# denix56/SI-Mamba

Hardware: AMD Instinct MI355X
Metric: point-clouds/sec (fwd+bwd) (higher is better)
Workload: dtype f32; 1 GPU; PointMamba classifier train step (FPS+kNN grouping, encoder, spectral SAST ordering, 12 Mamba blocks d=384 at L=1024, head, AdamW), 1024 pts -> 128 patches; global_batch=64, per_gpu_batch=64, npoints=1024, patches=128, mamba_seq_len=1024, parallelism=dp1, communicator_ranks=1, library_gemm=tuned solution table (si_mamba_amd/tuned/gemm_gfx950.csv)

## Files before the change

### include/simamba.h

```cpp
#ifndef SIMAMBA_H_
#define SIMAMBA_H_

#include <stddef.h>

#ifdef __cplusplus
extern "C" {
#endif

#define SIMAMBA_ABI_VERSION 9

#define SIMAMBA_F32  0
#define SIMAMBA_BF16 1

#define SIMAMBA_OK            0
#define SIMAMBA_E_NULLPTR    -1
#define SIMAMBA_E_SHAPE      -2
#define SIMAMBA_E_DTYPE      -3
#define SIMAMBA_E_DSTATE     -4
#define SIMAMBA_E_WIDTH      -5
#define SIMAMBA_E_WORKSPACE  -6
#define SIMAMBA_E_GROUPS     -7
#define SIMAMBA_E_ALIGN      -8
#define SIMAMBA_E_VARIANT    -9
#define SIMAMBA_E_BIAS       -10
// ... 44 lines not shown
                                  const float* delta_bias, const void* dout, const float* x_ckpt,
                                  void* du, void* ddelta, float* dA, float* dB, float* dC,
                                  float* dD, void* dz, float* ddelta_bias,
                                  int batch, int dim, int seqlen, int dstate,
                                  int io_dtype, int delta_softplus, long long z_bstride,
                                  long long dz_bstride, long long bc_bstride, long long bc_nstride,
                                  long long bc_tstride, int ckpt_step, int flags, float* workspace,
                                  long long workspace_floats, void* stream);

int simamba_selective_scan_dt_fwd(const void* u, const void* xdbl, const void* wdt, const float* A, const float* D,
                                  const void* z, const float* delta_bias, void* out, float* x_ckpt, float* last_state,
                                  int batch, int dim, int seqlen, int dstate, int dt_rank, int io_dtype,
                                  long long z_bstride, long long xdbl_bstride, long long xdbl_tstride, int ckpt_step,
                                  int variant, void* stream);
int simamba_selective_scan_dt_bwd(const void* u, const void* xdbl, const void* wdt, const float* A, const float* D,
                                  const void* z, const float* delta_bias, const void* dout, const float* x_ckpt,
                                  void* du, void* ddelta, float* dA, float* dB, float* dC, float* dD, void* dz,
                                  float* ddelta_bias, int batch, int dim, int seqlen, int dstate, int dt_rank,
                                  int io_dtype, long long z_bstride, long long dz_bstride, long long xdbl_bstride,
                                  long long xdbl_tstride, void* stream);
int simamba_selective_scan_dt_bwd_ex(const void* u, const void* xdbl, const void* wdt, const float* A, const float* D,
                                     const void* z, const float* delta_bias, const void* dout, const float* x_ckpt,
                                     void* du, void* ddelta, float* dA, float* dB, float* dC, float* dD, void* dz,
                                     float* ddelta_bias, int batch, int dim, int seqlen, int dstate, int dt_rank,
                                     int io_dtype, long long z_bstride, long long dz_bstride, long long xdbl_bstride,
                                     long long xdbl_tstride, int flags, float* workspace, long long workspace_floats,
                                     void* stream);

int simamba_xdt_proj_fwd(const void* x, const void* wx, const void* wdt, void* xdbl, void* delta,
                         int batch, int D, int seqlen, int S, int R, int io_dtype, long long x_bstride,
                         void* stream);
int simamba_conv_xdt_proj_fwd(const void* x, const float* cw, const float* cb, const void* wx, const void* wdt,
                              void* xconv, void* xdbl, void* delta, int batch, int D, int seqlen, int S, int R,
                              int io_dtype, long long x_bstride, void* stream);

int simamba_seq_gather_fwd(const void* in, const int* idx, void* out, int batch, int channels, int G, int L,
                           long long out_bstride, int io_dtype, void* stream);
int simamba_seq_gather_bwd(const void* dout, const int* inv, void* din, int batch, int channels, int G, int L,
                           int R, long long dout_bstride, int io_dtype, void* stream);

int simamba_causal_conv1d_fwd(const void* x, const float* w, const float* bias, void* out,
                              int batch, int dim, int seqlen, int width, int silu,
                              int io_dtype, long long x_bstride, void* stream);
int simamba_causal_conv1d_bwd(const void* x, const float* w, const float* bias,
                              const void* dout, void* dx, float* dw, float* dbias,
                              int batch, int dim, int seqlen, int width, int silu,
                              int io_dtype, long long x_bstride, long long dx_bstride, void* stream);
long long simamba_causal_conv1d_bwd_workspace_floats(int batch, int dim, int seqlen, int width, int flags);
int simamba_causal_conv1d_bwd_ex(const void* x, const float* w, const float* bias,
                                 const void* dout, void* dx, float* dw, float* dbias,
                                 int batch, int dim, int seqlen, int width, int silu,
                                 int io_dtype, long long x_bstride, long long dx_bstride, int flags,
                                 float* workspace, long long workspace_floats, void* stream);

int simamba_add_layer_norm_grid(int batch, int rows_per_batch);
int simamba_add_layer_norm_fwd(const void* hidden, const float* residual, const float* rowscale,
                               const float* weight, const float* bias, float* residual_out,
                               void* normed, float* mean, float* rstd, int batch, int rows_per_batch,
                               int dim, float eps, int hidden_dtype, int out_dtype, void* stream);
int simamba_add_layer_norm_bwd(const void* dnormed, const float* dresidual_out,
                               const float* residual_out, const float* mean, const float* rstd,
                               const float* weight, const float* rowscale, float* dresidual,
                               void* dhidden, float* dwb_partial, int batch, int rows_per_batch,
                               int dim, int hidden_dtype, int out_dtype, void* stream);

#define SIMAMBA_NORM_RMS 1
int simamba_add_layer_norm_fwd_ex(const void* hidden, const float* residual, const float* rowscale,
                                  const float* weight, const float* bias, float* residual_out,
                                  void* normed, float* mean, float* rstd, int batch, int rows_per_batch,
                                  int dim, float eps, int hidden_dtype, int out_dtype, int flags, void* stream);
int simamba_add_layer_norm_bwd_ex(const void* dnormed, const float* dresidual_out,
                                  const float* residual_out, const float* mean, const float* rstd,
                                  const float* weight, const float* rowscale, float* dresidual,
                                  void* dhidden, float* dwb_partial, int batch, int rows_per_batch,
                                  int dim, int hidden_dtype, int out_dtype, int flags, void* stream);

int simamba_add_layer_norm_check_slots(const int* slots_host, int batch, int compact_batch);
int simamba_add_layer_norm_fwd_slots(const void* hidden, const float* residual, const float* rowscale,
                                     const float* weight, const float* bias, float* residual_out,
                                     void* normed, float* mean, float* rstd, const int* hidden_slot,
                                     int hidden_batch, const int* normed_slot, int normed_batch, int batch,
                                     int rows_per_batch, int dim, float eps, int hidden_dtype, int out_dtype,
                                     int flags, void* stream);
int simamba_add_layer_norm_bwd_slots(const void* dnormed, const float* dresidual_out,
                                     const float* residual_out, const float* mean, const float* rstd,
                                     const float* weight, const float* rowscale, float* dresidual,
                                     void* dhidden, float* dwb_partial, const int* hidden_slot,
                                     int hidden_batch, const int* normed_slot, int normed_batch, int batch,
                                     int rows_per_batch, int dim, int hidden_dtype, int out_dtype, int flags,
                                     void* stream);

int simamba_out_proj_add_ln_fwd(const void* y, const void* w, const float* residual, const float* rowscale,
                                const float* gamma, const float* beta, float* residual_out, void* normed, float* mean,
                                float* rstd, int batch, int K, int L, int C, float eps, int out_dtype, void* stream);
int simamba_out_proj_add_ln_fwd_ex(const void* y, const void* w, const float* residual, const float* rowscale,
                                   const float* gamma, const float* beta, float* residual_out, void* normed,
                                   float* mean, float* rstd, int batch, int K, int L, int C, float eps, int out_dtype,
                                   int flags, void* stream);

int simamba_in_proj_fwd(const void* x, const void* w, void* xz, int batch, int L, int C, int M, int io_dtype,
                        void* stream);

int simamba_bn_relu_grid(long long rows);
int simamba_bn_relu_fwd(const void* x, const float* gterm, int group, const float* weight, const float* bias,
                        float* running_mean, float* running_var, float momentum, float eps, int training,
                        void* y, float* mean, float* invstd, float* partial, long long rows, int C,
// ... 212 lines not shown
```

### si_mamba_amd/_lib.py

```python
from __future__ import annotations

import ctypes
import os
from ctypes import c_char_p, c_float, c_int, c_longlong, c_size_t, c_uint, c_void_p

_HERE = os.path.dirname(os.path.abspath(__file__))
LIB_PATH = os.path.join(_HERE, "libsimamba_hip.so")

F32, BF16 = 0, 1

SPEC_SYMMETRIC = 0x01
SPEC_SELF_LOOP = 0x02
SPEC_BINARY = 0x04
SPEC_MATRIX_SYM = 0x08
SPEC_SMALLEST = 0x10
SPEC_SIGMA_MEAN = 0x20
SPEC_LARGE_G = 0x40
SPEC_MAX_G = 128
SPEC_MAX_G_LARGE = 512
CURVE_Z, CURVE_HILBERT, CURVE_TRANS, CURVE_Z_TRANS, CURVE_HILBERT_TRANS = 0, 1, 2, 2, 3
CURVE_BOX_CLOUD, CURVE_BOX_FIXED = 0, 1
CURVE_MAX_G, CURVE_MAX_K, CURVE_MAX_BITS = 8192, 8, 16

SCAN_AUTO, SCAN_ROWSCAN, SCAN_LPC2, SCAN_LPC4, SCAN_MIX = 0, 1, 2, 4, 6
# ... 10 lines not shown
DS_NONE, DS_UNIT_SPHERE = 0, 1
DS_STREAM_SHUFFLE, DS_STREAM_ROWS, DS_STREAM_CHOICE = 1, 2, 3
DS_MAX_POINTS = 8192
OPTIM_CHUNK = 4096
OPTIM_MAX_SEGMENTS, OPTIM_MAX_CHUNKS, OPTIM_MAX_GROUPS = 65536, 1 << 20, 256
OPTIM_ZERO_GRADS = 1

_P = c_void_p
_LL = c_longlong
ABI_VERSION = 9
SIGNATURES = {
    "simamba_abi_version": (c_int, []),
    "simamba_strerror": (c_char_p, [c_int]),
    "simamba_scan_num_chunks": (c_int, [c_int]),
    "simamba_scan_fwd_auto_variant": (c_int, [c_int, c_int]),
    "simamba_scan_ckpt_step": (c_int, [c_int, c_int, c_int, c_int, c_int]),
    "simamba_scan_ckpt_floats": (_LL, [c_int, c_int, c_int, c_int, c_int]),
    "simamba_scan_seq_applicable": (c_int, [c_int, c_int, c_int, c_int, c_int, c_int, c_int,
                                            c_size_t, c_size_t, c_size_t, c_size_t, _LL, _LL, _LL, _LL, _LL]),
    "simamba_selective_scan_fwd": (c_int, [_P, _P, _P, _P, _P, _P, _P, _P, _P, _P, _P,
                                           c_int, c_int, c_int, c_int, c_int, c_int,
                                           _LL, _LL, _LL, _LL, c_int, c_int, _P]),
    "simamba_selective_scan_bwd": (c_int, [_P, _P, _P, _P, _P, _P, _P, _P, _P, _P,
                                           _P, _P, _P, _P, _P, _P, _P, _P,
                                           c_int, c_int, c_int, c_int, c_int, c_int,
                                           _LL, _LL, _LL, _LL, _LL, c_int, _P]),
    "simamba_scan_bwd_workspace_floats": (_LL, [c_int, c_int, c_int, c_int, c_int, c_int]),
    "simamba_selective_scan_bwd_ex": (c_int, [_P, _P, _P, _P, _P, _P, _P, _P, _P, _P,
                                              _P, _P, _P, _P, _P, _P, _P, _P,
                                              c_int, c_int, c_int, c_int, c_int, c_int,
                                              _LL, _LL, _LL, _LL, _LL, c_int, c_int, _P, _LL, _P]),
    "simamba_selective_scan_dt_fwd": (c_int, [_P, _P, _P, _P, _P, _P, _P, _P, _P, _P,
                                              c_int, c_int, c_int, c_int, c_int, c_int,
                                              _LL, _LL, _LL, c_int, c_int, _P]),
    "simamba_selective_scan_dt_bwd": (c_int, [_P, _P, _P, _P, _P, _P, _P, _P, _P,
                                              _P, _P, _P, _P, _P, _P, _P, _P,
                                              c_int, c_int, c_int, c_int, c_int, c_int,
                                              _LL, _LL, _LL, _LL, _P]),
    "simamba_selective_scan_dt_bwd_ex": (c_int, [_P, _P, _P, _P, _P, _P, _P, _P, _P,
                                                 _P, _P, _P, _P, _P, _P, _P, _P,
                                                 c_int, c_int, c_int, c_int, c_int, c_int,
                                                 _LL, _LL, _LL, _LL, c_int, _P, _LL, _P]),
    "simamba_xdt_proj_fwd": (c_int, [_P, _P, _P, _P, _P, c_int, c_int, c_int, c_int, c_int, c_int, _LL, _P]),
    "simamba_conv_xdt_proj_fwd": (c_int, [_P, _P, _P, _P, _P, _P, _P, _P, c_int, c_int, c_int, c_int, c_int, c_int, _LL,
                                          _P]),
    "simamba_seq_gather_fwd": (c_int, [_P, _P, _P, c_int, c_int, c_int, c_int, _LL, c_int, _P]),
    "simamba_seq_gather_bwd": (c_int, [_P, _P, _P, c_int, c_int, c_int, c_int, c_int, _LL, c_int, _P]),
    "simamba_causal_conv1d_fwd": (c_int, [_P, _P, _P, _P, c_int, c_int, c_int, c_int, c_int, c_int, _LL, _P]),
    "simamba_causal_conv1d_bwd": (c_int, [_P, _P, _P, _P, _P, _P, _P,
                                          c_int, c_int, c_int, c_int, c_int, c_int, _LL, _LL, _P]),
    "simamba_causal_conv1d_bwd_workspace_floats": (_LL, [c_int, c_int, c_int, c_int, c_int]),
    "simamba_causal_conv1d_bwd_ex": (c_int, [_P, _P, _P, _P, _P, _P, _P,
                                             c_int, c_int, c_int, c_int, c_int, c_int, _LL, _LL, c_int, _P, _LL, _P]),
    "simamba_add_layer_norm_grid": (c_int, [c_int, c_int]),
    "simamba_add_layer_norm_fwd": (c_int, [_P, _P, _P, _P, _P, _P, _P, _P, _P, c_int, c_int, c_int, c_float,
                                           c_int, c_int, _P]),
    "simamba_add_layer_norm_bwd": (c_int, [_P, _P, _P, _P, _P, _P, _P, _P, _P, _P, c_int, c_int, c_int,
                                           c_int, c_int, _P]),
    "simamba_add_layer_norm_fwd_ex": (c_int, [_P, _P, _P, _P, _P, _P, _P, _P, _P, c_int, c_int, c_int, c_float,
                                              c_int, c_int, c_int, _P]),
    "simamba_add_layer_norm_bwd_ex": (c_int, [_P, _P, _P, _P, _P, _P, _P, _P, _P, _P, c_int, c_int, c_int,
                                              c_int, c_int, c_int, _P]),
    "simamba_add_layer_norm_check_slots": (c_int, [_P, c_int, c_int]),
    "simamba_add_layer_norm_fwd_slots": (c_int, [_P, _P, _P, _P, _P, _P, _P, _P, _P, _P, c_int, _P, c_int, c_int, c_int,
                                                 c_int, c_float, c_int, c_int, c_int, _P]),
    "simamba_add_layer_norm_bwd_slots": (c_int, [_P, _P, _P, _P, _P, _P, _P, _P, _P, _P, _P, c_int, _P, c_int, c_int,
                                                 c_int, c_int, c_int, c_int, c_int, _P]),
    "simamba_out_proj_add_ln_fwd": (c_int, [_P, _P, _P, _P, _P, _P, _P, _P, _P, _P, c_int, c_int, c_int, c_int, c_float,
                                            c_int, _P]),
    "simamba_out_proj_add_ln_fwd_ex": (c_int, [_P, _P, _P, _P, _P, _P, _P, _P, _P, _P, c_int, c_int, c_int, c_int,
                                               c_float, c_int, c_int, _P]),
    "simamba_in_proj_fwd": (c_int, [_P, _P, _P, c_int, c_int, c_int, c_int, c_int, _P]),
    "simamba_bn_relu_grid": (c_int, [_LL]),
    "simamba_bn_relu_fwd": (c_int, [_P, _P, c_int, _P, _P, _P, _P, c_float, c_float, c_int, _P, _P, _P, _P, _LL, c_int,
                                    _LL, c_int, _P]),
    "simamba_bn_relu_bwd": (c_int, [_P, _P, _P, c_int, _P, _P, _P, _P, _P, _P, c_int, _P, _P, _P, _LL, c_int, _LL,
                                    c_int, c_int, _P]),
    "simamba_bn_stats_local": (c_int, [_P, _P, c_int, _P, _LL, _P, _LL, c_int, _LL, c_int, _P]),
    "simamba_bn_stats_merge": (c_int, [_P, c_int, _P, _P, c_float, c_float, _P, _P, _P, c_int, _P]),
    "simamba_bn_relu_apply": (c_int, [_P, _P, c_int, _P, _P, _P, _P, _P, _LL, c_int, _LL, c_int, _P]),
    "simamba_bn_relu_bwd_sums": (c_int, [_P, _P, _P, c_int, _P, _P, _P, _P, _P, _P, _P, _LL, c_int, _LL, c_int, _P]),
    "simamba_bn_relu_bwd_dx": (c_int, [_P, _P, _P, c_int, _P, _P, _P, _P, _P, _P, _P, _P, _P, c_int, _LL, c_int, _LL,
                                       c_int, _P]),
    "simamba_group_max_fwd": (c_int, [_P, _P, _P, _LL, c_int, c_int, c_int, _P]),
    "simamba_group_max_bwd": (c_int, [_P, _P, _P, _LL, c_int, c_int, c_int, _P]),
    "simamba_max_linear_bwd_slabs": (c_int, [_LL, c_int]),
    "simamba_max_linear_bwd_dx": (c_int, [_P, _P, _P, _P, _LL, c_int, c_int, c_int, c_int, _P]),
    "simamba_max_linear_bwd_dw": (c_int, [_P, _P, _P, _P, _P, _LL, c_int, c_int, c_int, c_int, _P]),
    "simamba_three_nn": (c_int, [_P, _P, _P, _P, c_int, c_int, c_int, _P]),
    "simamba_three_interpolate_fwd": (c_int, [_P, _P, _P, _P, c_int, c_int, c_int, c_int, c_int, _P]),
    "simamba_three_interpolate_bwd": (c_int, [_P, _P, _P, _P, c_int, c_int, c_int, c_int, c_int, _P]),
    "simamba_gather_sum_scatter": (c_int, [_P, _P, _P, _P, c_int, c_int, c_int, c_int, c_int, c_int, _P]),
    "simamba_chamfer_fwd": (c_int, [_P, _P, _P, _P, _P, _LL, c_int, c_int, _P]),
    "simamba_chamfer_bwd": (c_int, [_P, _P, _P, _P, _P, _P, _LL, c_int, c_int, _P]),
    "simamba_chamfer_large_fwd": (c_int, [_P, _P, _P, _P, _P, _P, _P, _LL, c_int, c_int, _P]),
    "simamba_chamfer_large_bwd": (c_int, [_P, _P, _P, _P, _P, _P, _P, _LL, c_int, c_int, _P]),
    "simamba_chamfer_large_fwd_ex": (c_int, [_P, _P, _P, _P, _P, _P, _P, _LL, c_int, c_int, c_int, _P]),
    "simamba_chamfer_large_bwd_ex": (c_int, [_P, _P, _P, _P, _P, _P, _P, _LL, c_int, c_int, c_int, _P]),
    "simamba_chamfer_ragged_fwd": (c_int, [_P] * 9 + [_LL] + [c_int] * 6 + [_P]),
    "simamba_chamfer_ragged_bwd": (c_int, [_P] * 11 + [_LL] + [c_int] * 6 + [_P]),
    "simamba_emd_fwd": (c_int, [_P, _P, _P, _P, _P, _P, _LL, c_int, c_float, c_int, _P]),
    "simamba_sinkhorn_workspace_bytes": (c_size_t, [_LL, c_int, c_int, c_int]),
    "simamba_sinkhorn_fwd": (c_int, [_P] * 12 + [_LL, c_int, c_int, c_float, c_int, c_int, _P, c_size_t, _P]),
    "simamba_sinkhorn_bwd": (c_int, [_P] * 11 + [_LL, c_int, c_int, c_float, c_int, _P, c_size_t, _P]),
    "simamba_part_seg_eval": (c_int, [_P] * 12 + [_LL, c_int, c_int, c_int, _P]),
    "simamba_svm_ovo_fit": (c_int, [_P] * 10 + [c_int, c_int, c_int, c_int, c_int, _P]),
# ... 172 lines not shown
_scan_ckpt = [0]


class scan_ckpt(_Override):
    cell, coerce = _scan_ckpt, int

    def __init__(self, step):
        super().__init__(step)


_spectral_large_g = [False]


class spectral_large_g(_Override):
    cell = _spectral_large_g

    def __init__(self, on=True):
        super().__init__(on)


def spectral_large_g_forced():
    return _spectral_large_g[0]


_fuse_dt = [None]
counters = {}


def count(name):
    counters[name] = counters.get(name, 0) + 1


class scan_fuse_dt(_Override):
    cell, coerce = _fuse_dt, staticmethod(_tristate)


def fuse_dt_enabled(dtype):
    import torch
    return (dtype == torch.bfloat16) if _fuse_dt[0] is None else _fuse_dt[0]


_fuse_out_norm = [True]
_hand_in_proj = [None]


class fuse_out_norm(_Override):
    cell = _fuse_out_norm


def fuse_out_norm_enabled():
    return _fuse_out_norm[0]


_drop_path_compact = [os.environ.get("SIMAMBA_DROP_PATH_COMPACT", "1").strip().lower() not in ("0", "false", "off")]
DROP_PATH_BUCKET = 4
compact_sizes = {}


class drop_path_compact(_Override):
    cell = _drop_path_compact


def drop_path_compact_enabled():
    return _drop_path_compact[0]


_sparse_max_linear = [None]


class sparse_max_linear(_Override):
    cell, coerce = _sparse_max_linear, staticmethod(_tristate)


def sparse_max_linear_enabled(dtype):
    import torch
    return (dtype == torch.float32) if _sparse_max_linear[0] is None else _sparse_max_linear[0]


class hand_in_proj(_Override):
    cell, coerce = _hand_in_proj, staticmethod(_tristate)


def in_proj_hand_enabled(workgroups, dtype=None):
    import torch
    if _hand_in_proj[0] is not None:
        return _hand_in_proj[0]
    return dtype != torch.float32 and workgroups >= IN_PROJ_MIN_WORKGROUPS


IN_PROJ_MIN_WORKGROUPS = 192


def scan_plan_step(batch, dim, seqlen, dstate, dtype, *, softplus=True, has_z=True, act_addr_or=0, a_addr=0,
                   b_addr=0, c_addr=0, z_bs=0, dz_bs=0, bc_strides=(0, 0, 0)):
    lib = load()
    code = dtype_code(dtype)
    step = _scan_ckpt[0] or lib.simamba_scan_ckpt_step(batch, dim, seqlen, dstate, code)
    if step == CKPT_SEQ and not lib.simamba_scan_seq_applicable(
            batch, dim, seqlen, dstate, code, int(bool(softplus)), int(bool(has_z)), act_addr_or, a_addr, b_addr,
            c_addr, z_bs, dz_bs, *bc_strides):
        step = CKPT_ROW
    if _scan_variant[0] == SCAN_ROWSCAN:
        step = CKPT_ROW
    return step


# ... 59 lines not shown
```

### si_mamba_amd/add_norm.py

```python
from __future__ import annotations

import torch

from . import _lib


def add_norm_bwd(dn, dro, res_out, mean, rstd, w, rs, dres, dhid, Bsz, rows, dim, hcode, ocode, flags,
                 hidden_slot=None, hidden_batch=None, normed_slot=None, normed_batch=None):
    dev = res_out.device
    grid = _lib.load().simamba_add_layer_norm_grid(Bsz, rows)
    part = torch.empty(grid, 2, dim, device=dev, dtype=torch.float32)
    hb = Bsz if hidden_slot is None else hidden_batch
    nb = Bsz if normed_slot is None else normed_batch
    _lib.call("simamba_add_layer_norm_bwd_slots", dn, dro, res_out, mean, rstd, w, rs, dres, dhid, part, hidden_slot, hb,
              normed_slot, nb, Bsz, rows, dim, hcode, ocode, flags, device=dev,
              time_as="add_rms_bwd" if flags else "add_ln_bwd")
    return part[:, :1].sum(0) if flags else part.sum(0)


class AddLayerNormFn(torch.autograd.Function):
    @staticmethod
    def forward(ctx, hidden, residual, weight, bias, eps, rowscale, out_dtype, rms=False, hidden_slot=None,
                hidden_dtype=None, normed_slot=None, normed_batch=None):
        full = hidden if hidden_slot is None else residual
        if full is None:
            raise ValueError("add_layer_norm_fn: a compact hidden (hidden_slot) goes with a residual")
        _lib.require_gpu(full, "add_layer_norm_fn")
        h = None if hidden is None else hidden.contiguous()
        Bsz, rows, dim = full.shape[0], full[0].numel() // full.shape[-1], full.shape[-1]
        shape = tuple(full.shape)
        dev = full.device
        hdtype = h.dtype if h is not None else (hidden_dtype or torch.float32)
        hb = Bsz if hidden_slot is None else (0 if h is None else h.shape[0])
        nb = Bsz if normed_slot is None else int(normed_batch)
        if h is not None and tuple(h.shape[1:]) != shape[1:]:
            raise ValueError(f"add_layer_norm_fn: hidden {tuple(h.shape)} against residual {shape}")
        hcode = _lib.dtype_code(hdtype)
        ocode = _lib.dtype_code(out_dtype)
        flags = _lib.NORM_RMS if rms else 0
        res = None if residual is None else residual.float().contiguous()
        w = weight.float().contiguous()
        b = None if bias is None else bias.float().contiguous()
        rs = None if (rowscale is None or res is None) else rowscale.float().contiguous()
        alias = res is None and hdtype == torch.float32
        res_out = h if alias else torch.empty(shape, device=dev, dtype=torch.float32)
        normed = torch.empty((nb,) + shape[1:], device=dev, dtype=out_dtype)
        mean = None if rms else torch.empty(Bsz * rows, device=dev, dtype=torch.float32)
        rstd = torch.empty(Bsz * rows, device=dev, dtype=torch.float32)
        _lib.call("simamba_add_layer_norm_fwd_slots", h, res, rs, w, b, None if alias else res_out, normed, mean, rstd,
                  hidden_slot, hb, normed_slot, nb, Bsz, rows, dim, float(eps), hcode, ocode, flags, device=dev,
                  time_as="add_rms_fwd" if rms else "add_ln_fwd")
        ctx.save_for_backward(res_out, mean, rstd, w, rs, hidden_slot, normed_slot)
        ctx.meta = (Bsz, rows, dim, hcode, ocode, hdtype, residual is not None,
                    None if residual is None else residual.dtype, weight.dtype, bias is not None, flags, hb, nb)
        return normed, res_out

    @staticmethod
    def backward(ctx, dnormed, dres_out):
        res_out, mean, rstd, w, rs, hidden_slot, normed_slot = ctx.saved_tensors
        Bsz, rows, dim, hcode, ocode, hdtype, has_res, res_dtype, wdtype, has_bias, flags, hb, nb = ctx.meta
        dev = res_out.device
        dn = dnormed.contiguous()
        dro = None if dres_out is None else dres_out.float().contiguous()
        need_split = (rs is not None) or (hdtype != torch.float32) or not has_res or hidden_slot is not None
        dres = torch.empty(res_out.shape, device=dev, dtype=torch.float32) if has_res else None
        dhid = torch.empty((hb,) + tuple(res_out.shape[1:]), device=dev, dtype=hdtype) if need_split and hb else None
        dwb = add_norm_bwd(dn, dro, res_out, mean, rstd, w, rs, dres, dhid, Bsz, rows, dim, hcode, ocode, flags,
                           hidden_slot, hb, normed_slot, nb)
        if dhid is None and hidden_slot is None:
            dhid = dres
# ... 19 lines not shown
```

### si_mamba_amd/csrc/api.hip

```cpp
#include <hip/hip_runtime.h>

#include "../../include/simamba.h"

extern "C" int simamba_abi_version(void) { return SIMAMBA_ABI_VERSION; }

extern "C" const char* simamba_strerror(int rc) {
  switch (rc) {
    case SIMAMBA_OK: return "ok";
    case SIMAMBA_E_NULLPTR: return "simamba: required pointer is NULL";
    case SIMAMBA_E_SHAPE: return "simamba: bad shape (negative size, dim <= 0 or batch > 65535)";
    case SIMAMBA_E_DTYPE: return "simamba: io_dtype must be SIMAMBA_F32 or SIMAMBA_BF16";
    case SIMAMBA_E_DSTATE: return "simamba: dstate must be in [1,16]";
    case SIMAMBA_E_WIDTH: return "simamba: conv width must be in [2,4]";
    case SIMAMBA_E_WORKSPACE: return "simamba: workspace missing or too small";
    case SIMAMBA_E_GROUPS: return "simamba: need 2 <= G <= 128 (512 for the graph, _ex and fused calls), knn + 1 <= min(G, 32), k (+1) <= G (<= 8 above 128), 1 <= F <= 64";
    case SIMAMBA_E_ALIGN: return "simamba: pointer not aligned";
    case SIMAMBA_E_VARIANT: return "simamba: scan variant unknown or not applicable to this shape, unknown flag bits, or an augmentation chain / buffer overlap the call cannot take";
    case SIMAMBA_E_BIAS: return "simamba: SIMAMBA_NORM_RMS takes no bias / beta (pass NULL)";
    default: break;
  }
  if (rc > 0) return hipGetErrorString(static_cast<hipError_t>(rc));
  return "simamba: unknown error code";
}
```

### si_mamba_amd/csrc/det_reduce.h

```cpp
#pragma once
#include <hip/hip_runtime.h>

namespace simamba {

struct DetSumJob {
  const float* part;
  float* out;
  long long kstride;
  long long n;
  int K;
};

constexpr int kDetSumMaxJobs = 5;

int det_sum_launch(const DetSumJob* jobs, int njobs, hipStream_t s);

}
```

### si_mamba_amd/csrc/det_reduce.hip

```cpp
#include "det_reduce.h"

namespace simamba {

constexpr int kDetSumThreads = 256;
constexpr int kDetSumPerBlock = 4 * kDetSumThreads;

struct DetSumArgs {
  DetSumJob job[kDetSumMaxJobs];
  int vec[kDetSumMaxJobs];
  int blk0[kDetSumMaxJobs + 1];
  int njobs;
};

__global__ __launch_bounds__(kDetSumThreads) void det_sum_kernel(DetSumArgs a) {
  const int blk = blockIdx.x;
  int j = 0;
#pragma unroll
  for (int q = 1; q < kDetSumMaxJobs; ++q) j = (q < a.njobs && blk >= a.blk0[q]) ? q : j;
  const float* __restrict__ part = a.job[j].part;
  float* __restrict__ out = a.job[j].out;
  const long long ks = a.job[j].kstride, n = a.job[j].n;
  const int K = a.job[j].K;
  const long long i0 = (static_cast<long long>(blk - a.blk0[j]) * kDetSumThreads + threadIdx.x) * 4;
  if (i0 >= n) return;
  if (a.vec[j] && i0 + 4 <= n) {
    const float* p = part + i0;
    float4 acc = make_float4(0.f, 0.f, 0.f, 0.f);
    int k = 0;
    for (; k + 4 <= K; k += 4) {
      float4 v[4];
#pragma unroll
      for (int m = 0; m < 4; ++m) v[m] = *reinterpret_cast<const float4*>(p + (k + m) * ks);
#pragma unroll
      for (int m = 0; m < 4; ++m) {
        acc.x += v[m].x; acc.y += v[m].y; acc.z += v[m].z; acc.w += v[m].w;
      }
    }
    for (; k < K; ++k) {
      const float4 v = *reinterpret_cast<const float4*>(p + k * ks);
      acc.x += v.x; acc.y += v.y; acc.z += v.z; acc.w += v.w;
    }
    *reinterpret_cast<float4*>(out + i0) = acc;
    return;
  }
  for (long long i = i0; i < n && i < i0 + 4; ++i) {
    float acc = 0.f;
    for (int k = 0; k < K; ++k) acc += part[k * ks + i];
    out[i] = acc;
  }
}

int det_sum_launch(const DetSumJob* jobs, int njobs, hipStream_t s) {
  DetSumArgs a{};
  int blocks = 0, m = 0;
  for (int i = 0; i < njobs && m < kDetSumMaxJobs; ++i) {
    if (jobs[i].n <= 0) continue;
    a.job[m] = jobs[i];
    a.vec[m] = (reinterpret_cast<uintptr_t>(jobs[i].part) & 15u) == 0 && (reinterpret_cast<uintptr_t>(jobs[i].out) & 15u) == 0 &&
               jobs[i].kstride % 4 == 0;
    a.blk0[m] = blocks;
    blocks += static_cast<int>((jobs[i].n + kDetSumPerBlock - 1) / kDetSumPerBlock);
    ++m;
  }
  if (!m) return static_cast<int>(hipSuccess);
  a.njobs = m;
  for (int q = m; q <= kDetSumMaxJobs; ++q) a.blk0[q] = blocks;
  hipLaunchKernelGGL(det_sum_kernel, dim3(blocks), dim3(kDetSumThreads), 0, s, a);
  return static_cast<int>(hipGetLastError());
}

}
```

### si_mamba_amd/encoder_ops.py

```python
from __future__ import annotations

import torch
import torch.distributed as dist

from . import _lib


_BN_MAX_C = 1024
_BN_CHUNK = 256


_SPLITK = 64
_SPLITK_MIN_ROWS = 512


class TokenLinearFn(torch.autograd.Function):

    @staticmethod
    def forward(ctx, x, weight, bias):
        y = torch.nn.functional.linear(x, weight, bias)
        ctx.save_for_backward(x, weight)
        ctx.has_bias = bias is not None
        return y

    @staticmethod
    def backward(ctx, dy):
        x, weight = ctx.saved_tensors
        dy = dy.contiguous()
        io = dy.dtype
        rows, n_out = dy.shape
        dx = dw = db = None
        if ctx.needs_input_grad[0]:
            dx = (dy @ weight.to(io)).to(x.dtype)
        if ctx.needs_input_grad[1]:
            xc = x.to(io).contiguous()
            if rows % _SPLITK == 0 and rows // _SPLITK >= _SPLITK_MIN_ROWS:
                m = rows // _SPLITK
                a = dy.view(_SPLITK, m, n_out).transpose(1, 2)
                b = xc.view(_SPLITK, m, xc.shape[1])
                part = torch.bmm(a, b) if io == torch.float32 else torch.bmm(a, b, out_dtype=torch.float32)
                dw = part.sum(0).to(weight.dtype)
            else:
                dw = (dy.t() @ xc).to(weight.dtype)
        if ctx.has_bias and ctx.needs_input_grad[2]:
            db = dy.sum(0, dtype=torch.float32).to(weight.dtype)
        return dx, dw, db


def token_linear(x, weight, bias=None):
    if x.is_cuda and x.dim() == 2 and torch.is_grad_enabled() and (weight.requires_grad or x.requires_grad):
        return TokenLinearFn.apply(x, weight, bias)
    return torch.nn.functional.linear(x, weight, bias)


def _slices(C):
    return [(c0, min(c0 + _BN_MAX_C, C)) for c0 in range(0, C, _BN_MAX_C)]


def _off(t, elems):
    return None if t is None else t.data_ptr() + elems * t.element_size()


def _slice_of(g, c0, c1, C):
    return None if g is None else (g if (c0 == 0 and c1 == C) else g[:, c0:c1].contiguous())


def _bn_partial(lib, rows, C, dev):
    return torch.empty(lib.simamba_bn_relu_grid(rows), 2, min(C, _BN_MAX_C), device=dev, dtype=torch.float32)


def _bn_operands(x, gterm, weight, bias):
    xc = x.contiguous()
    g, w, b = (None if t is None else t.float().contiguous() for t in (gterm, weight, bias))
    mean = torch.empty(xc.shape[1], device=xc.device, dtype=torch.float32)
    return xc, g, w, b, torch.empty_like(xc), mean, torch.empty_like(mean)


def _dtypes(*tensors):
    return tuple(None if t is None else t.dtype for t in tensors)


def _bn_grads(dtypes, dx, dgt, dw, db):
    xdtype, gdtype, wdtype, bdtype = dtypes
    return (dx.to(xdtype), None if dgt is None else dgt.to(gdtype), None,
            None if wdtype is None else dw.to(wdtype), None if bdtype is None else db.to(bdtype),
            None, None, None, None, None)


def _bn_dgroup(g, group):
    dgroup = 0 if g is None else (group if _BN_CHUNK % group == 0 else _BN_CHUNK)
    if g is not None and dgroup == _BN_CHUNK and group % _BN_CHUNK != 0:
        raise ValueError("bn_relu_fn: group must divide 256 or be a multiple of it")
    return dgroup

# ... 298 lines not shown
```

### si_mamba_amd/mamba_inner.py

```python
from __future__ import annotations

import torch

from . import _lib


def _w(t, dtype):
    return t if t.dtype == dtype else t.to(dtype)


def _wx(W, X):
    return torch.bmm(W.unsqueeze(0).expand(X.shape[0], -1, -1), X)


def _xw(X, W):
    return torch.bmm(X, W.unsqueeze(0).expand(X.shape[0], -1, -1))


def _sum_bmm(X, Y):
    return torch.bmm(X, Y).sum(0, dtype=torch.float32)


class InProjFn(torch.autograd.Function):

    @staticmethod
    def forward(ctx, hidden, weight, bias):
        io = hidden.dtype
        if torch.is_autocast_enabled("cuda"):
            io = torch.get_autocast_dtype("cuda")
            hidden = hidden.to(io)
        wc = _w(weight, io)
        xz = tokens_times_weight(hidden, wc) if bias is None else _wx(wc, hidden.transpose(1, 2))
        if bias is not None:
            xz = xz + _w(bias, io)[None, :, None]
        ctx.save_for_backward(hidden, weight)
        ctx.wc = wc
        ctx.has_bias = bias is not None
        return xz

    @staticmethod
    def backward(ctx, dxz):
        hidden, weight = ctx.saved_tensors
        io = hidden.dtype
        dxz = dxz.to(io)
        dh = _xw(dxz.transpose(1, 2), ctx.wc) if ctx.needs_input_grad[0] else None
        dw = _sum_bmm(dxz, hidden).to(weight.dtype) if ctx.needs_input_grad[1] else None
        db = dxz.sum((0, 2)).to(weight.dtype) if ctx.has_bias else None
        return dh, dw, db


def tokens_times_weight(x, w):
    if (x.dtype in (torch.bfloat16, torch.float32) and w.dtype == x.dtype and x.is_cuda and x.dim() == 3
            and x.is_contiguous() and in_proj_hand_ok(x, w)):
        Bsz, L, C = x.shape
        wcc = w.contiguous()
        out = torch.empty(Bsz, w.shape[0], L, device=x.device, dtype=x.dtype)
        _lib.call("simamba_in_proj_fwd", x, wcc, out, Bsz, L, C, w.shape[0], _lib.dtype_code(x.dtype),
                  device=x.device, time_as="in_proj_fwd")
        _lib.count("in_proj_hand")
        return out
    return _wx(w, x.transpose(1, 2))


def in_proj_hand_ok(hidden, wc):
    Bsz, L, C = hidden.shape
    tile = 128 if hidden.dtype == torch.float32 else 256
    return (C % 64 == 0 and C <= 384 and wc.shape[0] % 32 == 0 and L % 8 == 0 and hidden.data_ptr() % 16 == 0
            and _lib.in_proj_hand_enabled(Bsz * ((L + tile - 1) // tile), hidden.dtype))


def in_proj_fn(hidden, weight, bias=None):
    return InProjFn.apply(hidden, weight, bias)

# ... 75 lines not shown
                x_dbl = _xw(x_conv.transpose(1, 2), xw_c.t())
                delta = _wx(dtw_c, x_dbl[:, :, :R].transpose(1, 2))
        Bv, Cv = x_dbl[:, :, R:R + N], x_dbl[:, :, R + N:]
        if x_dbl.data_ptr() % 16 or not x_dbl.is_contiguous():
            raise RuntimeError("mamba_inner_fn: x_proj output not as planned")

        y = torch.empty(Bsz, Dm, L, device=dev, dtype=io)
        dtw_k = dtw_c.contiguous() if fuse_dt else None
        if fuse_dt:
            _lib.count("scan_dt_fwd")
            _lib.call("simamba_selective_scan_dt_fwd", x_conv, x_dbl, dtw_k, Af, Df, z, bf, y, x_ckpt, None,
                      Bsz, Dm, L, N, R, code, xbs, x_dbl.stride(0), x_dbl.stride(1),
                      ckpt_step, _lib.current_scan_variant(), device=dev, time_as="scan_fwd")
        else:
            _lib.call("simamba_selective_scan_fwd", x_conv, delta, Af, Bv, Cv, Df, z, bf, y, x_ckpt, None,
                      Bsz, Dm, L, N, code, 1, xbs, x_dbl.stride(0), 1, x_dbl.stride(1),
                      ckpt_step, _lib.current_scan_variant(), device=dev, time_as="scan_fwd")

        if no_out:
            out = y
        else:
            out = _xw(y.transpose(1, 2), ow_c.t())
            if out_proj_b is not None:
                out = out + _w(out_proj_b, io)
        ctx.no_out = no_out
        ctx.dims = (R, N, W)
        ctx.ckpt_step = ckpt_step
        ctx.dtw_k = dtw_k
        ctx.has_out_bias = out_proj_b is not None and not no_out
        ctx.param_dtypes = (conv_w.dtype, None if conv_b is None else conv_b.dtype, x_proj_w.dtype,
                            dt_proj_w.dtype, None if no_out else out_proj_w.dtype, A.dtype,
                            None if D is None else D.dtype, None if delta_bias is None else delta_bias.dtype)
        ctx.save_for_backward(xz, x_conv, x_dbl, delta, None if no_out else y, cw, cb, x_proj_w, dt_proj_w, out_proj_w,
                              Af, Df, bf, x_ckpt)
        return out

    @staticmethod
    def backward(ctx, dout):
        (xz, x_conv, x_dbl, delta, y, cw, cb, x_proj_w, dt_proj_w, out_proj_w, Af, Df, bf, x_ckpt) = ctx.saved_tensors
        lib = _lib.load()
        R, N, W = ctx.dims
        io = xz.dtype
        code = _lib.dtype_code(io)
        Bsz, twoD, L = xz.shape
        Dm = twoD // 2
        S = R + 2 * N
        dev = xz.device
        xbs = xz.stride(0)
        dout = dout.to(io)
        f32 = dict(device=dev, dtype=torch.float32)
        xw_c, dtw_c, ow_c = ctx.wcast
        if ctx.no_out:
            dy = dout.contiguous()
            d_out_w = d_out_b = None
        else:
            if dout.stride(2) != 1:
                dout = dout.contiguous()
            d_out_w = _sum_bmm(dout.transpose(1, 2), y.transpose(1, 2))
            d_out_b = dout.sum((0, 1)) if ctx.has_out_bias else None
            dy = tokens_times_weight(dout, ow_c.t())

        dxz = torch.empty_like(xz)
        du = torch.empty(Bsz, Dm, L, device=dev, dtype=io)
        ddelta = torch.empty(Bsz, Dm, L, device=dev, dtype=io)
        dA, dB, dC, dD, dbias = _lib.scan_bwd_accumulators(Bsz, Dm, L, N, Df is not None, bf is not None, dev)
        Bv, Cv = x_dbl[:, :, R:R + N], x_dbl[:, :, R + N:]
        z, dz = xz[:, Dm:], dxz[:, Dm:]
        flags, ws, nws = _lib.det_args(lib.simamba_scan_bwd_workspace_floats, Bsz, Dm, L, N,
                                       _lib.CKPT_SEQ if ctx.dtw_k is not None else ctx.ckpt_step, device=dev)
        _lib.count("scan_bwd_det" if flags else "scan_bwd_atomic")
        if ctx.dtw_k is not None:
            _lib.call("simamba_selective_scan_dt_bwd_ex", x_conv, x_dbl, ctx.dtw_k, Af, Df, z, bf, dy, x_ckpt,
                      du, ddelta, dA, dB, dC, dD, dz, dbias, Bsz, Dm, L, N, R, code,
                      xbs, dxz.stride(0), x_dbl.stride(0), x_dbl.stride(1), flags, ws, nws,
                      device=dev, time_as="scan_bwd")
        else:
            _lib.call("simamba_selective_scan_bwd_ex", x_conv, delta, Af, Bv, Cv, Df, z, bf, dy, x_ckpt,
                      du, ddelta, dA, dB, dC, dD, dz, dbias, Bsz, Dm, L, N, code, 1,
                      xbs, dxz.stride(0), x_dbl.stride(0), 1, x_dbl.stride(1), ctx.ckpt_step, flags, ws, nws,
                      device=dev, time_as="scan_bwd")

        dx_dbl = torch.empty(Bsz, L, S, device=dev, dtype=io)
        dx_dbl[:, :, :R].copy_(_xw(ddelta.transpose(1, 2), dtw_c))
        dBC = torch.as_strided(dB, (2, Bsz, N, L), (Bsz * N * L, N * L, L, 1))
        dx_dbl[:, :, R:].view(Bsz, L, 2, N).copy_(dBC.permute(1, 3, 0, 2))
        d_dt_w = _sum_bmm(ddelta, x_dbl[:, :, :R])
        d_x_w = _sum_bmm(dx_dbl.transpose(1, 2), x_conv.transpose(1, 2))
        wxT = xw_c.t().unsqueeze(0).expand(Bsz, -1, -1)
        torch.baddbmm(du, wxT, dx_dbl.transpose(1, 2), out=du)

        dconv = torch.empty(Dm * W + (Dm if cb is not None else 0), **f32)
        dcw = dconv[:Dm * W].view(Dm, W)
        dcb = dconv[Dm * W:] if cb is not None else None
        flags, ws, nws = _lib.det_args(lib.simamba_causal_conv1d_bwd_workspace_floats, Bsz, Dm, L, W, device=dev)
        _lib.count("conv1d_bwd_det" if flags else "conv1d_bwd_atomic")
        _lib.call("simamba_causal_conv1d_bwd_ex", xz, cw, cb, du, dxz, dcw, dcb, Bsz, Dm, L, W, 1, code,
                  xbs, dxz.stride(0), flags, ws, nws, device=dev, time_as="conv1d_bwd")

        t_cw, t_cb, t_xw, t_dtw, t_ow, t_A, t_D, t_b = ctx.param_dtypes
        return (dxz, dcw.to(t_cw), None if dcb is None else dcb.to(t_cb), d_x_w.to(t_xw), d_dt_w.to(t_dtw),
                None if d_out_w is None else d_out_w.to(t_ow),
                None if d_out_b is None else d_out_b.to(out_proj_w.dtype), dA.to(t_A),
                None if dD is None else dD.to(t_D), None if dbias is None else dbias.to(t_b), None, None, None)


def mamba_inner_fn(xz, conv1d_weight, conv1d_bias, x_proj_weight, delta_proj_weight, out_proj_weight,
                   out_proj_bias, A, D=None, delta_bias=None, dt_rank=None, d_state=None):
    if conv1d_weight.dim() == 3:
        conv1d_weight = conv1d_weight.squeeze(1)
    if dt_rank is None:
        dt_rank = delta_proj_weight.shape[1]
    if d_state is None:
        d_state = (x_proj_weight.shape[0] - dt_rank) // 2
    return MambaInnerFn.apply(xz, conv1d_weight, conv1d_bias, x_proj_weight, delta_proj_weight, out_proj_weight,
                              out_proj_bias, A, D, delta_bias, dt_rank, d_state, torch.is_grad_enabled())
```

Measured before the change: 1177 point-clouds/s.

## Replace per-batch bmm partial sums with a fused multi-job deterministic batch_sum kernel

Adds a simamba_batch_sum entry point that reduces up to five per-batch partial tensors over the leading dimension in one launch, with f32/bf16 inputs and a split-K scheme that spreads each reduction across several threads followed by an LDS combine. The weight-gradient reductions in the mamba backward (out_proj, x_proj, dt_proj), the encoder split-K dw and the add-norm partials now call this kernel instead of separate torch sum calls. The aim is to cut launch count and use more of the GPU on these small reductions. It adds ctypes marshaling overhead on each call, and keeping p_out_w alive longer raises peak memory slightly.

```diff
diff --git a/include/simamba.h b/include/simamba.h
--- a/include/simamba.h
+++ b/include/simamba.h
@@ -120,6 +120,10 @@
                                  int batch, int dim, int seqlen, int width, int silu,
                                  int io_dtype, long long x_bstride, long long dx_bstride, int flags,
                                  float* workspace, long long workspace_floats, void* stream);
+
+#define SIMAMBA_BATCH_SUM_MAX_JOBS 5
+int simamba_batch_sum(const void* const* parts, float* const* outs, const long long* kstrides, const long long* ns,
+                      const int* Ks, const int* part_dtypes, int njobs, void* stream);
 
 int simamba_add_layer_norm_grid(int batch, int rows_per_batch);
 int simamba_add_layer_norm_fwd(const void* hidden, const float* residual, const float* rowscale,
diff --git a/si_mamba_amd/_lib.py b/si_mamba_amd/_lib.py
--- a/si_mamba_amd/_lib.py
+++ b/si_mamba_amd/_lib.py
@@ -86,6 +86,7 @@
     "simamba_causal_conv1d_bwd_workspace_floats": (_LL, [c_int, c_int, c_int, c_int, c_int]),
     "simamba_causal_conv1d_bwd_ex": (c_int, [_P, _P, _P, _P, _P, _P, _P,
                                              c_int, c_int, c_int, c_int, c_int, c_int, _LL, _LL, c_int, _P, _LL, _P]),
+    "simamba_batch_sum": (c_int, [_P, _P, _P, _P, _P, _P, c_int, _P]),
     "simamba_add_layer_norm_grid": (c_int, [c_int, c_int]),
     "simamba_add_layer_norm_fwd": (c_int, [_P, _P, _P, _P, _P, _P, _P, _P, _P, c_int, c_int, c_int, c_float,
                                            c_int, c_int, _P]),
@@ -364,6 +365,21 @@
     return _fuse_out_norm[0]
 
 
+_aten_batch_sum = [False]
+BATCH_SUM_MAX_JOBS = 5
+
+
+class aten_batch_sum(_Override):
+    cell = _aten_batch_sum
+
+    def __init__(self, on=True):
+        super().__init__(on)
+
+
+def aten_batch_sum_forced():
+    return _aten_batch_sum[0]
+
+
 _drop_path_compact = [os.environ.get("SIMAMBA_DROP_PATH_COMPACT", "1").strip().lower() not in ("0", "false", "off")]
 DROP_PATH_BUCKET = 4
 compact_sizes = {}
diff --git a/si_mamba_amd/add_norm.py b/si_mamba_amd/add_norm.py
--- a/si_mamba_amd/add_norm.py
+++ b/si_mamba_amd/add_norm.py
@@ -3,6 +3,7 @@
 import torch
 
 from . import _lib
+from .batch_sum import batch_sum
 
 
 def add_norm_bwd(dn, dro, res_out, mean, rstd, w, rs, dres, dhid, Bsz, rows, dim, hcode, ocode, flags,
@@ -15,7 +16,7 @@
     _lib.call("simamba_add_layer_norm_bwd_slots", dn, dro, res_out, mean, rstd, w, rs, dres, dhid, part, hidden_slot, hb,
               normed_slot, nb, Bsz, rows, dim, hcode, ocode, flags, device=dev,
               time_as="add_rms_bwd" if flags else "add_ln_bwd")
-    return part[:, :1].sum(0) if flags else part.sum(0)
+    return batch_sum([part[:, :1] if flags else part])[0]
 
 
 class AddLayerNormFn(torch.autograd.Function):
diff --git a/si_mamba_amd/batch_sum.py b/si_mamba_amd/batch_sum.py
--- /dev/null
+++ b/si_mamba_amd/batch_sum.py
@@ -0,0 +1,48 @@
+from __future__ import annotations
+
+import ctypes
+
+import torch
+
+from . import _lib
+
+
+_CODES = {torch.float32: _lib.F32, torch.bfloat16: _lib.BF16}
+_ARRAYS = {n: (ctypes.c_void_p * n, ctypes.c_longlong * n, ctypes.c_int * n)
+           for n in range(1, _lib.BATCH_SUM_MAX_JOBS + 1)}
+
+
+def _kernel_takes(part):
+    if not (part.is_cuda and part.dtype in _CODES and part.dim() >= 2):
+        return False
+    return part.is_contiguous() or part.shape[0] == 0 or part.select(0, 0).is_contiguous()
+
+
+def batch_sum(parts):
+    outs = [None] * len(parts)
+    jobs = []
+    for i, part in enumerate(parts):
+        if _lib.aten_batch_sum_forced():
+            _lib.count("batch_sum_aten")
+            outs[i] = part.sum(0, dtype=torch.float32)
+        elif not _kernel_takes(part):
+            outs[i] = part.sum(0, dtype=torch.float32)
+        else:
+            outs[i] = torch.empty(part.shape[1:], device=part.device, dtype=torch.float32)
+            jobs.append((part, outs[i]))
+    for j0 in range(0, len(jobs), _lib.BATCH_SUM_MAX_JOBS):
+        _launch(jobs[j0:j0 + _lib.BATCH_SUM_MAX_JOBS])
+    return outs
+
+
+def _launch(jobs):
+    n = len(jobs)
+    dev = jobs[0][0].device
+    if n > 1 and any(p.device != dev for p, _ in jobs):
+        raise ValueError("batch_sum: the partials of one call live on one device")
+    ptrs, longs, ints = _ARRAYS[n]
+    _lib.call("simamba_batch_sum",
+              ptrs(*[p.data_ptr() for p, _ in jobs]), ptrs(*[o.data_ptr() for _, o in jobs]),
+              longs(*[p.stride(0) if p.shape[0] > 1 else o.numel() for p, o in jobs]),
+              longs(*[o.numel() for _, o in jobs]), ints(*[p.shape[0] for p, _ in jobs]),
+              ints(*[_CODES[p.dtype] for p, _ in jobs]), n, device=dev)
diff --git a/si_mamba_amd/csrc/api.hip b/si_mamba_amd/csrc/api.hip
--- a/si_mamba_amd/csrc/api.hip
+++ b/si_mamba_amd/csrc/api.hip
@@ -13,7 +13,7 @@
     case SIMAMBA_E_DSTATE: return "simamba: dstate must be in [1,16]";
     case SIMAMBA_E_WIDTH: return "simamba: conv width must be in [2,4]";
     case SIMAMBA_E_WORKSPACE: return "simamba: workspace missing or too small";
-    case SIMAMBA_E_GROUPS: return "simamba: need 2 <= G <= 128 (512 for the graph, _ex and fused calls), knn + 1 <= min(G, 32), k (+1) <= G (<= 8 above 128), 1 <= F <= 64";
+    case SIMAMBA_E_GROUPS: return "simamba: need 2 <= G <= 128 (512 for the graph, _ex and fused calls), knn + 1 <= min(G, 32), k (+1) <= G (<= 8 above 128), 1 <= F <= 64; or 0 <= njobs <= 5 (simamba_batch_sum)";
     case SIMAMBA_E_ALIGN: return "simamba: pointer not aligned";
     case SIMAMBA_E_VARIANT: return "simamba: scan variant unknown or not applicable to this shape, unknown flag bits, or an augmentation chain / buffer overlap the call cannot take";
     case SIMAMBA_E_BIAS: return "simamba: SIMAMBA_NORM_RMS takes no bias / beta (pass NULL)";
diff --git a/si_mamba_amd/csrc/det_reduce.h b/si_mamba_amd/csrc/det_reduce.h
--- a/si_mamba_amd/csrc/det_reduce.h
+++ b/si_mamba_amd/csrc/det_reduce.h
@@ -4,14 +4,49 @@
 namespace simamba {
 
 struct DetSumJob {
-  const float* part;
+  const void* part;
   float* out;
   long long kstride;
   long long n;
   int K;
+  int split = 1;
+  int bf16 = 0;
 };
 
 constexpr int kDetSumMaxJobs = 5;
+constexpr int kDetSumMaxSplit = 16;
+constexpr long long kDetSumFillThreads = 256 * 1024;
+
+inline int det_sum_split(int K, long long n) {
+  const long long quads = (n + 3) / 4;
+  int s = 1;
+  while (s < kDetSumMaxSplit && quads * s < kDetSumFillThreads && K >= 8 * s) s *= 2;
+  return s;
+}
+
+constexpr int kDetSumThreads = 256;
+
+struct DetSumGrid {
+  int blk0[kDetSumMaxJobs + 1];
+  int used;
+  long long total;
+};
+
+inline long long det_sum_outputs_per_block(int split) { return 4LL * (kDetSumThreads / split); }
+
+inline DetSumGrid det_sum_grid(const DetSumJob* jobs, int njobs) {
+  DetSumGrid g{};
+  long long blocks = 0;
+  for (int i = 0; i < njobs && g.used < kDetSumMaxJobs; ++i) {
+    if (jobs[i].n <= 0) continue;
+    const long long per = det_sum_outputs_per_block(jobs[i].split);
+    g.blk0[g.used++] = static_cast<int>(blocks);
+    blocks += (jobs[i].n + per - 1) / per;
+  }
+  for (int q = g.used; q <= kDetSumMaxJobs; ++q) g.blk0[q] = static_cast<int>(blocks);
+  g.total = blocks;
+  return g;
+}
 
 int det_sum_launch(const DetSumJob* jobs, int njobs, hipStream_t s);
 
diff --git a/si_mamba_amd/csrc/det_reduce.hip b/si_mamba_amd/csrc/det_reduce.hip
--- a/si_mamba_amd/csrc/det_reduce.hip
+++ b/si_mamba_amd/csrc/det_reduce.hip
@@ -1,9 +1,8 @@
 #include "det_reduce.h"
 
+#include "../../include/simamba.h"
+
 namespace simamba {
-
-constexpr int kDetSumThreads = 256;
-constexpr int kDetSumPerBlock = 4 * kDetSumThreads;
 
 struct DetSumArgs {
   DetSumJob job[kDetSumMaxJobs];
@@ -12,61 +11,150 @@
   int njobs;
 };
 
+template <bool kBf16>
+__device__ __forceinline__ float4 det_load4(const void* p) {
+  if constexpr (kBf16) {
+    const uint2 r = *reinterpret_cast<const uint2*>(p);
+    return make_float4(__uint_as_float(r.x << 16), __uint_as_float(r.x & 0xffff0000u), __uint_as_float(r.y << 16),
+                       __uint_as_float(r.y & 0xffff0000u));
+  } else {
+    return *reinterpret_cast<const float4*>(p);
+  }
+}
+
+template <bool kBf16>
+__device__ __forceinline__ float det_load1(const void* p, long long i) {
+  if constexpr (kBf16) {
+    return __uint_as_float(static_cast<unsigned>(static_cast<const unsigned short*>(p)[i]) << 16);
+  } else {
+    return static_cast<const float*>(p)[i];
+  }
+}
+
+__device__ __forceinline__ void det_add(float4& acc, const float4& v) {
+  acc.x += v.x; acc.y += v.y; acc.z += v.z; acc.w += v.w;
+}
+
+template <bool kBf16>
+__device__ __forceinline__ float4 det_sum_range(const void* part, long long i0, long long ks, int k0, int k1, bool vec,
+                                                int lanes) {
+  float4 acc = make_float4(0.f, 0.f, 0.f, 0.f);
+  if (vec) {
+    constexpr int esz = kBf16 ? 2 : 4;
+    const char* p = static_cast<const char*>(part) + i0 * esz;
+    const long long kb = ks * esz;
+    int k = k0;
+    for (; k + 8 <= k1; k += 8) {
+      float4 v[8];
+#pragma unroll
+      for (int m = 0; m < 8; ++m) v[m] = det_load4<kBf16>(p + (k + m) * kb);
+#pragma unroll
+      for (int m = 0; m < 8; ++m) det_add(acc, v[m]);
+    }
+    if (k + 4 <= k1) {
+      float4 v[4];
+#pragma unroll
+      for (int m = 0; m < 4; ++m) v[m] = det_load4<kBf16>(p + (k + m) * kb);
+#pragma unroll
+      for (int m = 0; m < 4; ++m) det_add(acc, v[m]);
+      k += 4;
+    }
+    for (; k < k1; ++k) det_add(acc, det_load4<kBf16>(p + k * kb));
+    return acc;
+  }
+  for (int k = k0; k < k1; ++k) {
+    const long long o = k * ks + i0;
+    acc.x += det_load1<kBf16>(part, o);
+    if (lanes > 1) acc.y += det_load1<kBf16>(part, o + 1);
+    if (lanes > 2) acc.z += det_load1<kBf16>(part, o + 2);
+    if (lanes > 3) acc.w += det_load1<kBf16>(part, o + 3);
+  }
+  return acc;
+}
+
 __global__ __launch_bounds__(kDetSumThreads) void det_sum_kernel(DetSumArgs a) {
+  __shared__ float4 red[kDetSumThreads];
   const int blk = blockIdx.x;
   int j = 0;
 #pragma unroll
   for (int q = 1; q < kDetSumMaxJobs; ++q) j = (q < a.njobs && blk >= a.blk0[q]) ? q : j;
-  const float* __restrict__ part = a.job[j].part;
+  const void* __restrict__ part = a.job[j].part;
   float* __restrict__ out = a.job[j].out;
   const long long ks = a.job[j].kstride, n = a.job[j].n;
-  const int K = a.job[j].K;
-  const long long i0 = (static_cast<long long>(blk - a.blk0[j]) * kDetSumThreads + threadIdx.x) * 4;
-  if (i0 >= n) return;
-  if (a.vec[j] && i0 + 4 <= n) {
-    const float* p = part + i0;
-    float4 acc = make_float4(0.f, 0.f, 0.f, 0.f);
-    int k = 0;
-    for (; k + 4 <= K; k += 4) {
-      float4 v[4];
-#pragma unroll
-      for (int m = 0; m < 4; ++m) v[m] = *reinterpret_cast<const float4*>(p + (k + m) * ks);
-#pragma unroll
-      for (int m = 0; m < 4; ++m) {
-        acc.x += v[m].x; acc.y += v[m].y; acc.z += v[m].z; acc.w += v[m].w;
-      }
-    }
-    for (; k < K; ++k) {
-      const float4 v = *reinterpret_cast<const float4*>(p + k * ks);
-      acc.x += v.x; acc.y += v.y; acc.z += v.z; acc.w += v.w;
-    }
+  const int K = a.job[j].K, S = a.job[j].split;
+  const int qpb = kDetSumThreads / S;
+  const int tid = threadIdx.x;
+  const int r = tid / qpb, q = tid - r * qpb;
+  const long long i0 = (static_cast<long long>(blk - a.blk0[j]) * qpb + q) * 4;
+  const bool live = i0 < n;
+  const int lanes = live ? static_cast<int>(n - i0 < 4 ? n - i0 : 4) : 0;
+  const bool vec = a.vec[j] && lanes == 4;
+  const int len = (K + S - 1) / S;
+  const int k0 = r * len < K ? r * len : K;
+  const int k1 = k0 + len < K ? k0 + len : K;
+  float4 acc = make_float4(0.f, 0.f, 0.f, 0.f);
+  if (live) {
+    acc = a.job[j].bf16 ? det_sum_range<true>(part, i0, ks, k0, k1, vec, lanes)
+                        : det_sum_range<false>(part, i0, ks, k0, k1, vec, lanes);
+  }
+  if (S > 1) {
+    red[tid] = acc;
+    __syncthreads();
+    if (r != 0) return;
+    for (int p = 1; p < S; ++p) det_add(acc, red[p * qpb + q]);
+  }
+  if (!live) return;
+  if (vec) {
     *reinterpret_cast<float4*>(out + i0) = acc;
     return;
   }
-  for (long long i = i0; i < n && i < i0 + 4; ++i) {
-    float acc = 0.f;
-    for (int k = 0; k < K; ++k) acc += part[k * ks + i];
-    out[i] = acc;
-  }
+  out[i0] = acc.x;
+  if (lanes > 1) out[i0 + 1] = acc.y;
+  if (lanes > 2) out[i0 + 2] = acc.z;
+  if (lanes > 3) out[i0 + 3] = acc.w;
 }
 
 int det_sum_launch(const DetSumJob* jobs, int njobs, hipStream_t s) {
+  const DetSumGrid g = det_sum_grid(jobs, njobs);
+  if (!g.used) return static_cast<int>(hipSuccess);
+  if (g.total > 0x7fffffffLL) return static_cast<int>(hipErrorInvalidValue);
   DetSumArgs a{};
-  int blocks = 0, m = 0;
-  for (int i = 0; i < njobs && m < kDetSumMaxJobs; ++i) {
+  int m = 0;
+  for (int i = 0; i < njobs && m < g.used; ++i) {
     if (jobs[i].n <= 0) continue;
     a.job[m] = jobs[i];
-    a.vec[m] = (reinterpret_cast<uintptr_t>(jobs[i].part) & 15u) == 0 && (reinterpret_cast<uintptr_t>(jobs[i].out) & 15u) == 0 &&
+    const uintptr_t pa = jobs[i].bf16 ? 7u : 15u;
+    a.vec[m] = (reinterpret_cast<uintptr_t>(jobs[i].part) & pa) == 0 && (reinterpret_cast<uintptr_t>(jobs[i].out) & 15u) == 0 &&
                jobs[i].kstride % 4 == 0;
-    a.blk0[m] = blocks;
-    blocks += static_cast<int>((jobs[i].n + kDetSumPerBlock - 1) / kDetSumPerBlock);
     ++m;
   }
-  if (!m) return static_cast<int>(hipSuccess);
+  for (int q = 0; q <= kDetSumMaxJobs; ++q) a.blk0[q] = g.blk0[q];
   a.njobs = m;
-  for (int q = m; q <= kDetSumMaxJobs; ++q) a.blk0[q] = blocks;
-  hipLaunchKernelGGL(det_sum_kernel, dim3(blocks), dim3(kDetSumThreads), 0, s, a);
+  hipLaunchKernelGGL(det_sum_kernel, dim3(static_cast<unsigned>(g.total)), dim3(kDetSumThreads), 0, s, a);
   return static_cast<int>(hipGetLastError());
 }
 
 }
+
+extern "C" int simamba_batch_sum(const void* const* parts, float* const* outs, const long long* kstrides,
+                                 const long long* ns, const int* Ks, const int* part_dtypes, int njobs, void* stream) {
+  using namespace simamba;
+  static_assert(SIMAMBA_BATCH_SUM_MAX_JOBS == kDetSumMaxJobs, "the header's job limit is the launcher's");
+  if (njobs < 0 || njobs > kDetSumMaxJobs) return SIMAMBA_E_GROUPS;
+  if (njobs == 0) return SIMAMBA_OK;
+  if (!parts || !outs || !kstrides || !ns || !Ks || !part_dtypes) return SIMAMBA_E_NULLPTR;
+  DetSumJob jobs[kDetSumMaxJobs];
+  for (int i = 0; i < njobs; ++i) {
+    if (ns[i] < 0 || Ks[i] < 0 || kstrides[i] < 0) return SIMAMBA_E_SHAPE;
+    if (part_dtypes[i] != SIMAMBA_F32 && part_dtypes[i] != SIMAMBA_BF16) return SIMAMBA_E_DTYPE;
+    if (ns[i] > 0 && (!outs[i] || (Ks[i] > 0 && !parts[i]))) return SIMAMBA_E_NULLPTR;
+    jobs[i].part = parts[i];
+    jobs[i].out = outs[i];
+    jobs[i].kstride = kstrides[i];
+    jobs[i].n = ns[i];
+    jobs[i].K = Ks[i];
+    jobs[i].split = det_sum_split(Ks[i], ns[i]);
+    jobs[i].bf16 = part_dtypes[i] == SIMAMBA_BF16;
+  }
+  return det_sum_launch(jobs, njobs, static_cast<hipStream_t>(stream));
+}
diff --git a/si_mamba_amd/encoder_ops.py b/si_mamba_amd/encoder_ops.py
--- a/si_mamba_amd/encoder_ops.py
+++ b/si_mamba_amd/encoder_ops.py
@@ -4,6 +4,7 @@
 import torch.distributed as dist
 
 from . import _lib
+from .batch_sum import batch_sum
 
 
 _BN_MAX_C = 1024
@@ -39,7 +40,7 @@
                 a = dy.view(_SPLITK, m, n_out).transpose(1, 2)
                 b = xc.view(_SPLITK, m, xc.shape[1])
                 part = torch.bmm(a, b) if io == torch.float32 else torch.bmm(a, b, out_dtype=torch.float32)
-                dw = part.sum(0).to(weight.dtype)
+                dw = batch_sum([part])[0].to(weight.dtype)
             else:
                 dw = (dy.t() @ xc).to(weight.dtype)
         if ctx.has_bias and ctx.needs_input_grad[2]:
diff --git a/si_mamba_amd/mamba_inner.py b/si_mamba_amd/mamba_inner.py
--- a/si_mamba_amd/mamba_inner.py
+++ b/si_mamba_amd/mamba_inner.py
@@ -3,6 +3,7 @@
 import torch
 
 from . import _lib
+from .batch_sum import batch_sum
 
 
 def _w(t, dtype):
@@ -18,7 +19,7 @@
 
 
 def _sum_bmm(X, Y):
-    return torch.bmm(X, Y).sum(0, dtype=torch.float32)
+    return batch_sum([torch.bmm(X, Y)])[0]
 
 
 class InProjFn(torch.autograd.Function):
@@ -200,11 +201,11 @@
         xw_c, dtw_c, ow_c = ctx.wcast
         if ctx.no_out:
             dy = dout.contiguous()
-            d_out_w = d_out_b = None
+            p_out_w = d_out_b = None
         else:
             if dout.stride(2) != 1:
                 dout = dout.contiguous()
-            d_out_w = _sum_bmm(dout.transpose(1, 2), y.transpose(1, 2))
+            p_out_w = torch.bmm(dout.transpose(1, 2), y.transpose(1, 2))
             d_out_b = dout.sum((0, 1)) if ctx.has_out_bias else None
             dy = tokens_times_weight(dout, ow_c.t())
 
@@ -232,8 +233,9 @@
         dx_dbl[:, :, :R].copy_(_xw(ddelta.transpose(1, 2), dtw_c))
         dBC = torch.as_strided(dB, (2, Bsz, N, L), (Bsz * N * L, N * L, L, 1))
         dx_dbl[:, :, R:].view(Bsz, L, 2, N).copy_(dBC.permute(1, 3, 0, 2))
-        d_dt_w = _sum_bmm(ddelta, x_dbl[:, :, :R])
-        d_x_w = _sum_bmm(dx_dbl.transpose(1, 2), x_conv.transpose(1, 2))
+        partials = [torch.bmm(ddelta, x_dbl[:, :, :R]), torch.bmm(dx_dbl.transpose(1, 2), x_conv.transpose(1, 2))]
+        d_dt_w, d_x_w, *rest = batch_sum(partials + ([] if p_out_w is None else [p_out_w]))
+        d_out_w = rest[0] if rest else None
         wxT = xw_c.t().unsqueeze(0).expand(Bsz, -1, -1)
         torch.baddbmm(du, wxT, dx_dbl.transpose(1, 2), out=du)
 
```

After: 1183 point-clouds/s (median of 6 runs). No clear change (+0.5%).
